# pharaofranz/frb-baseband

Hardware: AMD Instinct MI355X
Metric: Msamples/s channelised to .fil per GPU; achieved HBM GB/s vs peak (higher is better)
Workload: dtype f32

## Files before the change

### frb_baseband_amd/csrc/frbch_api.cpp

```cpp
#include "frbch_internal.h"

namespace frbchi {
int settle_user_stream(frbch_handle* h) {
  if (h->user_stream) {
    h->user_stream = 0;
    if (h->user_ev_made && dev_event_sync(h->user_ev) != 0)
      return fail(h, FRBCH_E_DEVICE, std::string("sync (caller stream): ") + dev_last_error_string());
  }
  return FRBCH_OK;
}
void mark_user_stream(frbch_handle* h, dev_stream_t s) {
  if (!h->user_ev_made) {
    if (dev_event_create_sync(&h->user_ev) != 0) return;
    h->user_ev_made = true;
  }
  dev_event_record(h->user_ev, s);
  h->user_stream = s;
}
int enter_stream(frbch_handle* h, dev_stream_t s) {
  if (h->user_stream && h->user_stream != s) { const int rc = settle_user_stream(h); if (rc) return rc; }
  join_reset(h, s);
  return FRBCH_OK;
}
void leave_stream(frbch_handle* h, dev_stream_t s) { mark_user_stream(h, s); }
// ... 18 lines not shown
  if ((cfg->flags & kFlagBuffered) && (cfg->flags & kFlagTwoPass)) return fail(h, FRBCH_E_ARG, "cfg.flags asks for the buffered AND the two-pass rescale");
  {
    const uint32_t mode = (cfg->overlap >> 24) & 0xFFu, batches = (cfg->overlap >> 16) & 0xFFu;
    if ((mode != 0 && mode != 3) || batches)
      return fail(h, FRBCH_E_ARG, "cfg.overlap: only mode 3 (or 0) and no batch count are accepted (include/frbch.h)");
  }
  h->device = cfg->device;
  DeviceGuard dg(h->device);
  char arch[128] = "";
  if (!dev_arch_ok(h->device, arch, sizeof arch, &h->lds_limit)) return fail(h, FRBCH_E_DEVICE, "cannot query device");
  h->lane_ncu = dev_cu_count(h->device);
  if (h->cfg.unpack_mode == 1) h->cfg.flags |= kFlagGenericK1;
  const std::string why = make_plan(h->cfg, &h->pl, h->lds_limit);
  if (!why.empty()) return fail(h, FRBCH_E_ARG, why);
  const Plan& pl = h->pl;
  CHECK_DEV(h, dev_stream_create(&h->stream), "hipStreamCreate");
  int rc;
  if ((rc = upload_table(h, &h->tw_r, pl.r, std::max(1, pl.r / 2), 1))) return rc;
  if ((rc = upload_table(h, &h->tw_c2, pl.c2, pl.c, 1))) return rc;
  const uint64_t nlo = 1ull << pl.log2_nlo, nhi = pl.n >> pl.log2_nlo;
  if ((rc = upload_table(h, &h->tw_nlo, pl.n, nlo, 1))) return rc;
  if ((rc = upload_table(h, &h->tw_nhi, pl.n, std::max<uint64_t>(1, nhi), nlo))) return rc;
  if ((rc = apply_plan(h))) return rc;
  CHECK_DEV(h, dev_malloc((void**)&h->s_dc, (size_t)pl.maxb * pl.c2 * sizeof(cf)), "hipMalloc(s_dc)");
  CHECK_DEV(h, dev_malloc((void**)&h->p0, (size_t)pl.maxb * pl.c2 * sizeof(cf)), "hipMalloc(p0)");
  if (pl.dls_lg_ns) {
    const std::vector<float> tab = dls_table(1u << pl.dls_lg_ns, h->cfg.dls_cutoff_sigma, h->cfg.dls_threshold);
    CHECK_DEV(h, dev_malloc((void**)&h->dls_tab, tab.size() * sizeof(float)), "hipMalloc(level table)");
    CHECK_DEV(h, dev_h2d(h->dls_tab, tab.data(), tab.size() * sizeof(float), h->stream), "upload level table");
    CHECK_DEV(h, dev_sync(h->stream), "sync");
    h->dls_cap = (((uint64_t)pl.maxb - 1) * pl.hop + pl.n) >> pl.dls_lg_ns;
    CHECK_DEV(h, dev_malloc((void**)&h->dls_nlow, h->dls_cap * sizeof(uint32_t)), "hipMalloc(window counts)");
  }
  CHECK_DEV(h, dev_malloc((void**)&h->offset, pl.ncol * sizeof(float)), "hipMalloc(offset)");
  CHECK_DEV(h, dev_malloc((void**)&h->scale, pl.ncol * sizeof(float)), "hipMalloc(scale)");
  if ((rc = set_identity_rescale(h))) return rc;
  if (pl.interval_rows == 0) {
    h->have_scale = true;
    h->scale_frozen = true;
  }
  return FRBCH_OK;
}

extern "C" void frbch_close(frbch_handle* h) {
  if (!h) return;
  DeviceGuard dg(h->device);
  (void)settle_user_stream(h);
  if (h->stream) (void)dev_sync(h->stream);
  drain_events(h);
  dev_free(h->tw_r); dev_free(h->tw_c2); dev_free(h->tw_nhi); dev_free(h->tw_nlo);
  dev_free(h->ftw1_r); dev_free(h->ftw2_r); dev_free(h->ftw1_c); dev_free(h->ftw2_c); dev_free(h->td1); dev_free(h->td2);
  dev_free(h->spill); dev_free(h->s_dc); dev_free(h->p0);
  dev_free(h->spill2); dev_free(h->chirp); dev_free(h->ptmp); dev_free(h->scr2);
  dev_free(h->offset); dev_free(h->scale); dev_free(h->powbuf); dev_free(h->partial);
  dev_free(h->d_frames); dev_free(h->d_out); dev_free(h->stg); dev_free(h->d_fbad); dev_free(h->scan_rows);
  dev_free(h->dls_tab); dev_free(h->dls_nlow);
  for (int i = 0; i < 8; ++i) { dev_host_free(h->pin_in[i]); dev_host_free(h->pin_out[i]); }
  if (h->stream) dev_stream_destroy(h->stream);
  if (h->user_ev_made) dev_event_destroy(h->user_ev);
  if (h->quant_ev_made) dev_event_destroy(h->quant_ev);
  if (h->reset_ev_made) dev_event_destroy(h->reset_ev);
  if (h->spill_ev_made) dev_event_destroy(h->spill_ev);
  for (auto& e : h->evpool) dev_event_destroy(e);
  delete h;
}

extern "C" const char* frbch_last_error(frbch_handle* h) { return h ? h->err.c_str() : "null handle"; }

extern "C" int frbch_get_info(frbch_handle* h, frbch_info* info) {
  if (!h || !info) return FRBCH_E_ARG;
  const Plan& pl = h->pl;
  memset(info, 0, sizeof *info);
  info->size = (uint32_t)sizeof *info;
  info->nchan = pl.c; info->freq_res = pl.r; info->tscrunch = pl.tscr; info->nif = pl.nif;
  info->block_samples = pl.n;
  info->block_payload_bytes = pl.block_payload_bytes;
  info->rows_per_block = pl.rows_per_block;
  info->row_bytes = pl.row_bytes;
  info->rescale_interval_rows = pl.interval_rows;
  info->rows_out = h->rows_out;
  info->blocks_done = h->blocks_done;
  info->tsamp_s = pl.tsamp_s;
  info->tstart_mjd = h->tstart_mjd;
  info->fch1_mhz = pl.fch1; info->foff_mhz = pl.foff;
  info->frame_bytes = h->have_vdif ? h->v0.frame_bytes : 0;
  info->header_bytes = h->have_vdif ? h->v0.header_bytes() : 0;
  info->have_rescale = h->have_scale ? 1 : 0;
  info->diag = h->diag;
  info->frames_seen = h->frames_seen;
  info->frames_invalid = h->frames_invalid;
  info->frame_gaps = h->frame_gaps;
  info->frames_filled = h->frames_filled;
  info->block_stride_bytes = pl.block_stride_bytes;
  info->nfilt_pos = (uint32_t)pl.nfilt_pos;
  info->nfilt_neg = (uint32_t)pl.nfilt_neg;
  return FRBCH_OK;
}

extern "C" int frbch_reset(frbch_handle* h) {
  if (!h) return FRBCH_E_ARG;
  DeviceGuard dg(h->device);
  { const int rc = settle_user_stream(h); if (rc) return rc; }
  CHECK_DEV(h, dev_sync(h->stream), "sync");
  h->pow_rows = 0;
  h->fused_rows = 0;
  h->fused_valid = false;
  h->deferred.active = false;
// ... 242 lines not shown
```

### frb_baseband_amd/csrc/frbch_internal.h

```cpp
#ifndef FRBCH_INTERNAL_H
#define FRBCH_INTERNAL_H
#include FRBCH_DEV_HEADER

#include <errno.h>
#include <fcntl.h>
#include <math.h>
#include <stdio.h>
#include <stdlib.h>
#include <string.h>
#include <sys/mman.h>
#include <sys/stat.h>
#include <sys/uio.h>
#include <time.h>
#include <unistd.h>

#include <algorithm>
#include <atomic>
#include <chrono>
#include <sstream>
#include <string>
#include <condition_variable>
#include <map>
#include <mutex>
#include <thread>
#include <vector>

#include "frbch_host.h"
#include "frbch_kparams.h"

using namespace frbch;

enum { KID_K1 = 0, KID_KC, KID_K2, KID_STATS, KID_QUANT, KID_K3, KID_K4, KID_K0, KID_K2S, KID_K2P, KID_COUNT };
const char* const kKernelNames[KID_COUNT] = {"frbch_k1_branch", "frbch_kc_dcfix", "frbch_k2_chan",
                                             "frbch_stats", "frbch_quantise", "frbch_k3_dedisp", "frbch_k4_out", "frbch_k0_stage",
                                             "frbch_k2_statpass", "frbch_k2_priv"};
static_assert(KID_COUNT <= (int)(sizeof(((frbch_timing*)nullptr)->k) / sizeof(((frbch_timing*)nullptr)->k[0])), "frbch_timing holds every slot");

struct EventPair {
  dev_event_t a, b;
  int kid;
  double bytes;
};

struct frbch_handle {
  frbch_config cfg;
  Plan pl;
  std::string err;
  int device = 0;
  dev_stream_t stream = 0;
  dev_stream_t user_stream = 0;
  dev_event_t user_ev{};
  bool user_ev_made = false;
  size_t lds_limit = 65536;

  cf *tw_r = nullptr, *tw_c2 = nullptr, *tw_nhi = nullptr, *tw_nlo = nullptr;
  cf *ftw1_r = nullptr, *ftw2_r = nullptr, *ftw1_c = nullptr, *ftw2_c = nullptr, *td1 = nullptr, *td2 = nullptr;
  cf *spill = nullptr, *s_dc = nullptr, *p0 = nullptr;
  cf *spill2 = nullptr, *chirp = nullptr;
  int coh_order_m = 0;
  float* ptmp = nullptr;
  float *offset = nullptr, *scale = nullptr;
  bool have_scale = false;
  bool scale_frozen = false;
  float* powbuf = nullptr;
  float* scr2 = nullptr;
  uint64_t pow_cap_rows = 0, pow_rows = 0;
  double* partial = nullptr;
  int partial_chunks = 0;
  uint64_t fused_rows = 0;
  bool fused_valid = false;
  int fused_chunks = 0;
  int fused_live = 0;

  uint64_t rows_out = 0, blocks_done = 0;
  struct Deferred {
    bool active = false;
    KParams p;
    uint32_t nb = 0;
    uint64_t rows = 0;
  } deferred;
  int priv_grid = 0;

  bool have_vdif = false;
  VdifInfo v0{};
  double tstart_mjd = 0.0;
  uint64_t skip_bytes = 0;
  uint64_t blocks_budget = 0;
  std::vector<uint8_t> carry;
  uint64_t frames_seen = 0, frames_invalid = 0, frame_gaps = 0, frames_filled = 0;
  std::vector<uint8_t> carry_bad;
  uint32_t* d_fbad = nullptr;
  float* dls_tab = nullptr;
  uint32_t* dls_nlow = nullptr;
  uint64_t dls_cap = 0;
  size_t d_fbad_words = 0;
  uint64_t next_frame_index = 0;
  size_t checked_bytes = 0;
  uint8_t* d_frames = nullptr;
  size_t d_frames_cap = 0;
  uint8_t* d_out = nullptr;
  size_t d_out_cap = 0;
  uint8_t* stg = nullptr;
  bool stg_ready = false;
  std::vector<uint8_t> outq;
  size_t outq_pos = 0;
  uint8_t* pin_in[8] = {nullptr, nullptr, nullptr, nullptr, nullptr, nullptr, nullptr, nullptr};
  uint8_t* pin_out[8] = {nullptr, nullptr, nullptr, nullptr, nullptr, nullptr, nullptr, nullptr};
  size_t pin_in_cap = 0, pin_out_cap = 0;
  uint8_t* sink = nullptr;
  size_t sink_line_pitch = 0;
  uint64_t sink_rows = 0, sink_rows_cap = 0;

  uint64_t out_pitch = 0;
  int lane_cus = 0;
  int lane_ncu = 0;
  bool quant_lds_allowed = false;
  dev_event_t spill_ev{};
  bool spill_ev_made = false, spill_busy = false;
  std::vector<dev_event_t> evpool;
  size_t evnext = 0;
  uint32_t diag = 0;
// ... 164 lines not shown
```

### frb_baseband_amd/csrc/frbch_kparams.h

```cpp
#ifndef FRBCH_KPARAMS_H
#define FRBCH_KPARAMS_H
#include <stdint.h>

struct __attribute__((aligned(8))) cf {
  float x, y;
};

struct __attribute__((aligned(16))) f4 {
  float v[4];
};

enum { FRBCH_OUT_FLOAT_POWER = 0, FRBCH_OUT_CODES = 1,
       FRBCH_OUT_STATS = 2 };

struct KParams {
  int log2_c2;
  int log2_r;
  int c;
  int c2;
  int r;
  int g;
  int tt;
  int tscr;
  int nif;
  int pol_mode;
  int nbit;
  int flip;
  int out_mode;
  int log2_nlo;
  int log2_g;
  int in_bits;
  uint32_t frame_bytes, header_bytes, payload_bytes;
  uint32_t rel0;
  uint64_t payload_off;
  const uint8_t* frames;
  uint64_t gs;
  cf* spill;
  cf* s_dc;
  cf* p0;
  const cf* tw_r;
  const cf* tw_c2;
  const cf* tw_nhi;
  const cf* tw_nlo;
  const cf* ftw1_r;
  const cf* ftw2_r;
  const cf* ftw1_c;
  const cf* ftw2_c;
  const cf* td1;
  const cf* td2;
  const float* offset;
  const float* scale;
  float* power_out;
  uint8_t* code_out;
  uint64_t row0;
  uint64_t out_pitch;
  uint32_t div_magic, div_shift;
  float lut[4];
  float digi_mean, digi_scale, digi_max;
  cf rot6[6];
  int coherent;
  int nfilt_pos;
  int keep;
  uint64_t hop;
  cf* spill2;
  const cf* chirp;
  float* ptmp;
  const float* scr_in;
  uint32_t scr_fact;
  uint64_t scr_rows;
  double* stat_partial;
  uint64_t stat_limit;
  uint32_t nblk;
  uint32_t stat_first;
  const uint8_t* stg;
  uint8_t* stg_out;
  int tile_major;
  const uint32_t* fbad;
  uint64_t fbad_frame0;
  uint32_t* dls_nlow;
  const float* dls_tab;
  int dls_lg_ns;
};

struct StatParams {
  const float* power;
  double* partial;
  uint64_t rows;
  uint64_t rows_per_chunk;
  int ncol, c, nif, flip, nchunk;
  int rsplit;
  int cpw;
  float* offset;
  float* scale;
};

struct QuantParams {
  const float* power;
  uint8_t* out;
  uint64_t rows;
  int ncol, c, nif, flip, nbit;
  const float* offset;
  const float* scale;
  float digi_mean, digi_scale, digi_max;
  uint32_t grid_x;
  int log2_c;
  int log2_ncol;
  uint64_t pitch;
  uint32_t rphases;
};
#define QUANT_GRID_X(p) ((p).grid_x)

struct ChirpParams {
  cf* chirp;
  int c, c2, r, log2_r;
  int usb;
  int order_m;
  double band_edge_mhz;
  double df_mhz;
  double dm_over_k;
};

#define FRBCH_CODE_INDEX(pitch, row, nif, prod, cout) ((((uint64_t)(row)) * (uint64_t)(nif) + (uint64_t)(prod)) * (uint64_t)(pitch) + (uint64_t)(cout))

#define S2_INDEX(row, pos, r) (((((uint64_t)(row) >> 2) * (uint64_t)(r) + (uint64_t)(pos)) << 2) + (uint64_t)((row) & 3))

#endif
// ... 1 lines not shown
```

### frb_baseband_amd/csrc/frbch_launch.cpp

```cpp
#include "frbch_internal.h"

#include "kernels_generic.inc"
#ifndef FRBCH_NO_FAST
#include "kernels_fast.inc"
#include "kernels_k2priv.inc"
#endif

namespace frbchi {

int upload_table(frbch_handle* h, cf** dst, uint64_t n, uint64_t count, uint64_t step) {
  std::vector<float> tmp(2 * count);
  fill_twiddles(tmp.data(), n, count, step);
  CHECK_DEV(h, dev_malloc((void**)dst, count * sizeof(cf)), "hipMalloc(twiddles)");
  CHECK_DEV(h, dev_h2d(*dst, tmp.data(), count * sizeof(cf), h->stream), "upload twiddles");
  CHECK_DEV(h, dev_sync(h->stream), "sync");
  return FRBCH_OK;
}

KParams base_params(const frbch_handle* h) {
  const Plan& pl = h->pl;
  KParams p;
  memset(&p, 0, sizeof p);
  p.log2_c2 = pl.log2_c2;
  p.log2_r = pl.log2_r;
// ... 192 lines not shown
  }
}
template <class F>
bool select_k2_fast(const Plan& pl, F&& f) {
  if (pl.fast_k2_log2m != 5) return false;
  if (pl.fast_k2_nt == 512) f(fast::frbch_k2_fast<5, 512>, ksel(512, pl.k2_fast_lds, "frbch_k2_fast", {5, 512}));
  else f(fast::frbch_k2_fast<5, 1024>, ksel(1024, pl.k2_fast_lds, "frbch_k2_fast", {5, 1024}));
  return true;
}
template <class F>
bool select_k2c_fast(const Plan& pl, F&& f) {
  return on_value<1, 2, 3, 4, 5>(pl.coh_fast_c, [&](auto L) {
    f(fast::frbch_k2c_fast<L.value, 1024>, ksel(1024, pl.k2c_fast_lds, "frbch_k2c_fast").with({L.value, 1024}));
  });
}
constexpr uint32_t kK3WaveWgs = 2048;
bool k3_wave_planned(const Plan& pl) {
  return pl.coherent && pl.coh_fast_r == 4 && pl.coh_nt == 512;
}
template <class F>
bool select_k3_fast(const Plan& pl, F&& f) {
  if (pl.coh_nt == 512) {
    if (!k3_wave_planned(pl)) return false;
    f(fast::frbch_k3_wave<4>, ksel(256, pl.k3_fast_lds, "frbch_k3_wave", {4}));
    return true;
  }
  return on_value<1, 2, 3, 5>(pl.coh_fast_r, [&](auto L) {
    f(fast::frbch_k3_fast<L.value, 1024>, ksel(1024, pl.k3_fast_lds, "frbch_k3_fast").with({L.value, 1024}));
  });
}
bool k4_fast_planned(const Plan& pl, uint32_t h_flags) {
  return pl.ncol % 64 == 0 && pl.rows_per_block % 2 == 0 && pl.c % 4 == 0 && !(h_flags & kFlagGenericK2);
}

constexpr uint32_t kFusedStatWgs = 2048;
int priv_stat_chunks(const Plan& pl, int grid) { return grid * (pl.ncol / 4 >= 256 ? 1 : (int)(256 / (pl.ncol / 4))); }
bool pol_mode_no_sums(int pol_mode) { return pol_mode == 3; }
bool priv_takes(const Plan& pl, const KParams& p, int priv_grid) {
  return pl.fast_k2_priv && p.tile_major == 2 && priv_grid > 0 &&
         !(p.out_mode == FRBCH_OUT_FLOAT_POWER && pl.fast_k2_nw == 2 && pl.fast_k2_log2m == 3);
}
struct PrivLaunch {
  unsigned grid;
  bool sums;
};
PrivLaunch priv_launch(const frbch_handle* h, const KParams& p, uint32_t nb) {
  const Plan& pl = h->pl;
  if (pl.fast_k2_lane || !priv_takes(pl, p, h->priv_grid)) return {0u, false};
  const uint64_t ntiles = (uint64_t)nb * (uint64_t)(pl.r / 4);
  const bool sums = p.stat_partial && k2_wave_planned(pl) && !pl.coherent &&
                    !pol_mode_no_sums(p.pol_mode) && !(h->cfg.flags & kFlagSeparateStats);
  return {(unsigned)std::min<uint64_t>(ntiles, (uint64_t)h->priv_grid), sums};
}
int wave_stat_chunks(const Plan& pl, uint32_t h_flags, int pol_mode) {
  if (pol_mode_no_sums(pol_mode) || pl.k2_two_stage) return 0;
  if (k3_wave_planned(pl)) return (h_flags & kFlagSeparateStats) ? 0 : (int)kK3WaveWgs;
  if (!k2_wave_planned(pl) || pl.coherent || (h_flags & kFlagSeparateStats)) return 0;
  int nt = 0;
  select_k2_wave(pl, pol_mode, false, [&](auto, const KSel& a) { nt = a.nt; });
  const int cg = (int)(pl.ncol / 4);
  if (!nt) return 0;
  if (cg > nt)
    return (cg % nt == 0 && cg / nt <= 4)
               ? (pl.fast_k2_log2m == 5 ? 256 : ((pl.fast_k2_log2m == 3 && pl.fast_k2_nw != 8) ? (int)kFusedStatWgs : 0))
               : 0;
  if (nt % cg != 0) return 0;
  return (int)kFusedStatWgs * (nt / cg);
}
int fused_stat_chunks(const Plan& pl, uint32_t h_flags, int pol_mode, int priv_grid = 0) {
  const int w = wave_stat_chunks(pl, h_flags, pol_mode);
  if (pol_mode_no_sums(pol_mode) || pl.k2_two_stage || (h_flags & kFlagSeparateStats)) return w;
  return (pl.fast_k2_priv && priv_grid > 0) ? std::max(w, priv_stat_chunks(pl, priv_grid)) : w;
}

void set_fastdiv(KParams& p) {
  const uint32_t d = p.payload_bytes;
  uint32_t l = 0;
  while ((1ull << l) < d) ++l;
  p.div_magic = (uint32_t)((((1ull << l) - d) << 32) / d + 1);
  p.div_shift = l ? l - 1 : 0;
}
bool launch_k1_wave(frbch_handle* h, KParams& p, uint32_t nb, dev_stream_t s, int ncu) {
  const Plan& pl = h->pl;
  p.nblk = nb;
  const int kg = pl.fast_k1_g;
  {
    static const int ks[6] = {1, 2, 3, 4, 8, 12};
    const int step = 64 / kg;
    for (int i = 0; i < 6; ++i) {
      const double a = -2.0 * M_PI * (double)((step * ks[i]) % pl.r) / (double)pl.r;
      p.rot6[i].x = (float)cos(a);
      p.rot6[i].y = (float)sin(a);
    }
  }
  const uint32_t ngrp = (uint32_t)(pl.c2 / kg);
  const uint32_t resident = (uint32_t)(ncu > 0 ? ncu : 256) * (uint32_t)std::max<size_t>(1, (160 * 1024) / pl.k1_fast_lds);
  uint32_t ny = std::max<uint32_t>(1, std::min<uint32_t>(nb, resident / std::max<uint32_t>(1, ngrp)));
  if (ngrp > resident && ngrp % resident != 0) {
    uint32_t g = ngrp, r = resident;
    while (r) { const uint32_t t = g % r; g = r; r = t; }
    const uint32_t want = resident / g;
    if (want <= nb) ny = want;
  }
  return select_k1_wave(pl, p.stg != nullptr, p.fbad != nullptr, [&](auto kern, const KSel& a) { launch_sel(h, kern, dim3(ngrp, ny), a, s, p); });
}
bool launch_k2_wave(frbch_handle* h, KParams& p, uint32_t nb, dev_stream_t s, uint32_t h_flags) {
// ... 47 lines not shown
  if (!pl.fast_k1_log2m) return false;
  const uint32_t rb = (uint32_t)(pl.fast_k1_wave ? pl.fast_k1_g : pl.g) / 2;
  if (p.payload_off % rb || p.payload_bytes % rb || p.header_bytes % rb || p.frame_bytes % rb ||
      ((uintptr_t)p.frames % 16))
    return false;
  if (pl.fast_k1_wave) {
    if (p.payload_bytes < 2) return false;
    const uint64_t fr0 = p.payload_off / p.payload_bytes;
    const uint64_t rel0 = p.payload_off - fr0 * p.payload_bytes;
    if (rel0 + (uint64_t)nb * pl.block_payload_bytes >= (1ull << 32)) return false;
    KParams q = p;
    q.frames = p.frames + fr0 * p.frame_bytes;
    q.rel0 = (uint32_t)rel0;
    set_fastdiv(q);
    if (h->stg_ready) q.stg = h->stg;
    h->stg_ready = false;
    if (p.fbad) {
      if (!q.stg || k1_wave_lds(pl, true) > h->lds_limit) return false;
      q.fbad_frame0 = p.fbad_frame0 + fr0;
    }
    q.tile_major = p.tile_major = pl.spill_tile_major;
    return launch_k1_wave(h, q, nb, s, h->lane_cus);
  }
  p.tile_major = pl.spill_tile_major == 8 ? 8 : 0;
  KParams q = p;
  if (h->stg_ready) q.stg = h->stg;
  h->stg_ready = false;
  {
    const uint64_t fr0 = p.payload_off / p.payload_bytes;
    const uint64_t rel0 = p.payload_off - fr0 * p.payload_bytes;
    const uint64_t span = rel0 + (uint64_t)(nb - 1) * pl.block_stride_bytes + pl.block_payload_bytes;
    if (p.payload_bytes >= 2 && span < (1ull << 32)) {
      q.frames = p.frames + fr0 * p.frame_bytes;
      q.rel0 = (uint32_t)rel0;
      q.payload_off = rel0;
      set_fastdiv(q);
    } else {
      q.div_magic = 0;
    }
  }
  return select_k1_fast(pl, [&](auto kern, const KSel& a) { launch_sel(h, kern, dim3(pl.c2 / pl.g, nb), a, s, q); });
}
bool launch_k2_fast(frbch_handle* h, KParams& p, uint32_t nb, dev_stream_t s) {
  const Plan& pl = h->pl;
  if (pl.fast_k2_lane) {
    if (p.tile_major) return false;
    const dim3 grid((unsigned)((uint64_t)pl.r * nb * pl.fast_k2_lane / 256));
    return select_k2_lane(pl, p.pol_mode, [&](auto kern, const KSel& a) { launch_sel(h, kern, grid, a, s, p); });
  }
  if (const PrivLaunch pv = priv_launch(h, p, nb); pv.grid) {
    p.nblk = nb;
    if (!pv.sums) p.stat_partial = nullptr;
    if (!p.stat_partial) p.stat_first = 0;
    const dim3 grid(pv.grid);
    return select_k2_priv(pl, p.pol_mode, p.out_mode, [&](auto kern, const KSel& a) { launch_sel(h, kern, grid, a, s, p); });
  }
  if (p.out_mode == FRBCH_OUT_STATS) return false;
  if (!pl.fast_k2_wave && pl.fast_k2_log2m != 5) return false;
  KParams q = p;
  if (pl.k2_two_stage) {
    q.tscr = pl.k2_stage1_tscr;
    q.out_mode = FRBCH_OUT_FLOAT_POWER;
    q.power_out = h->scr2;
    q.row0 = 0;
    q.stat_partial = nullptr;
  }
  KParams& k = pl.k2_two_stage ? q : p;
  if (pl.fast_k2_wave) {
    if (!launch_k2_wave(h, k, nb, s, h->cfg.flags)) return false;
  } else {
    select_k2_fast(pl, [&](auto kern, const KSel& a) {
      launch_sel(h, kern, dim3(pl.r / (a.nt == 512 ? 1 : std::max(2, k.tscr)), nb), a, s, k);
    });
  }
  if (pl.k2_two_stage) {
    p.scr_in = h->scr2;
    p.scr_fact = (uint32_t)pl.k2_two_stage;
    p.scr_rows = (uint64_t)nb * pl.rows_per_block;
    p.stat_partial = nullptr;
    const uint64_t groups = p.scr_rows * (uint64_t)(pl.ncol / 4);
    const unsigned gx = (unsigned)std::min<uint64_t>((groups + 255) / 256, 8192);
    if (h->profiling) note_launch(h, "frbch_k2_scrunch", gx, 1);
    hipLaunchKernelGGL(fast::frbch_k2_scrunch, dim3(gx), dim3(256), 0, s, p);
  }
  return true;
}
bool launch_k2c_fast(frbch_handle* h, KParams& p, uint32_t nb, dev_stream_t s) {
  const Plan& pl = h->pl;
  if (!pl.coh_fast_c) return false;
  const int tt = 1024 / (16 << pl.coh_fast_c);
  p.nblk = nb;
  const uint32_t ntile = (uint32_t)(pl.r / tt);
  const uint32_t want = 4u * (uint32_t)std::max(1, h->lane_ncu);
  const uint32_t gy = std::max<uint32_t>(1, std::min<uint32_t>(nb, (want + ntile - 1) / ntile));
  return select_k2c_fast(pl, [&](auto kern, const KSel& a) { launch_sel(h, kern, dim3(ntile, gy), a, s, p); });
}
bool launch_k3_fast(frbch_handle* h, KParams& p, uint32_t nb, dev_stream_t s) {
  const Plan& pl = h->pl;
  if (!pl.coh_fast_r || !h->coh_order_m) return false;
  if (k3_wave_planned(pl)) {
    const uint64_t ntiles = (uint64_t)nb * pl.c;
    return select_k3_fast(pl, [&](auto kern, const KSel& a) {
      p.nblk = nb;
      launch_sel(h, kern, dim3((unsigned)std::min<uint64_t>(ntiles, kK3WaveWgs)), a, s, p);
    });
  }
// ... 141 lines not shown
  const Plan& pl = h->pl;
  p.tile_major = 0;
  if (pl.dls_lg_ns) {
    const int rc = launch_dls_count(h, p, ((uint64_t)nb - 1) * pl.hop + pl.n, s);
    if (rc) return rc;
  }
  {
    const bool masked = p.fbad != nullptr;
    if (!masked || pl.fast_k1_wave) launch_k0_stage(h, p, nb, s);
    const double bytes = (double)nb * ((double)pl.block_payload_bytes * p.frame_bytes / p.payload_bytes +
                                       (double)pl.n * 8.0 + (double)pl.c2 * 8.0);
    ProfScope ps(h, s, KID_K1, bytes);
    bool done = false;
    if (masked && !(pl.fast_k1_wave && (!pl.coherent || h->coh_order_m) && (done = launch_k1_fast(h, p, nb, s)))) {
      h->stg_ready = false;
      if (pl.coherent && h->coh_order_m) {
        const int rc = build_chirp(h, 0);
        if (rc) return rc;
      }
    } else if (masked) {
    } else if (!pl.coherent) done = launch_k1_fast(h, p, nb, s);
    else if (h->coh_order_m) {
      done = launch_k1_fast(h, p, nb, s);
      if (!done) {
        const int rc = build_chirp(h, 0);
        if (rc) return rc;
      }
    }
    if (!done) {
      REC_LAUNCH(h, frbch_k1_branch, pl.c2 / pl.g, nb, pl.nthreads, pl.k1_lds, s, p);
      if (!h->kname[KID_K1].empty() && h->kname[KID_K1].find(kKernelNames[KID_K1]) == std::string::npos)
        h->kname[KID_K1] += std::string("+") + kKernelNames[KID_K1];
    }
  }
  if (!pl.coherent) {
    ProfScope ps(h, s, KID_KC, (double)nb * pl.c2 * 16.0);
    if (!launch_kc_fast(h, p, nb, s)) REC_LAUNCH(h, frbch_kc_dcfix, 1, nb, pl.nthreads, pl.kc_lds, s, p);
  }
  CHECK_DEV(h, dev_check_launch(), "launch K1/Kc");
  return FRBCH_OK;
}

int launch_back(frbch_handle* h, KParams& p, uint32_t nb, dev_stream_t s) {
  const Plan& pl = h->pl;
  const int tile_t = std::max(pl.tt, pl.tscr);
  const double out_b = p.out_mode == FRBCH_OUT_FLOAT_POWER ? (double)pl.ncol * 4.0 : (double)pl.row_bytes;
  const double bytes = (double)nb * ((double)pl.n * 8.0 + (double)pl.rows_per_block * out_b);
#ifndef FRBCH_NO_FAST
  const bool k3_sums = k3_wave_planned(pl) && h->coh_order_m != 0;
#else
  const bool k3_sums = false;
#endif
  if ((!k2_wave_planned(pl) || pl.coherent) && !k3_sums) p.stat_partial = nullptr;
  if (p.out_mode == FRBCH_OUT_STATS) {
    ProfScope ps(h, s, KID_K2S, (double)nb * (double)pl.n * 8.0);
    if (!launch_k2_fast(h, p, nb, s)) return fail(h, FRBCH_E_STATE, "statistics-only K2 pass without frbch_k2_priv");
    CHECK_DEV(h, dev_check_launch(), "launch K2 (statistics pass)");
    return FRBCH_OK;
  }
  if (pl.coherent) {
    {
      ProfScope ps(h, s, KID_K2, ((double)nb * 16.0 + (pl.coh_fast_c ? 1.0 : (double)nb) * 8.0) * (double)pl.n);
      if (!launch_k2c_fast(h, p, nb, s)) REC_LAUNCH(h, frbch_k2c_chirp, pl.r / pl.tt, nb, pl.nthreads, pl.k2_lds, s, p);
    }
    {
      ProfScope ps(h, s, KID_K3, (double)nb * ((double)pl.n * 8.0 + (double)pl.rows_per_block * pl.ncol * 4.0));
      if (!launch_k3_fast(h, p, nb, s)) REC_LAUNCH(h, frbch_k3_dedisp, pl.c, nb, pl.nthreads, pl.k3_lds, s, p);
    }
    {
      ProfScope ps(h, s, KID_K4, (double)nb * (double)pl.rows_per_block * (pl.ncol * 4.0 + out_b));
      const int tc = pl.ncol < 64 ? (int)pl.ncol : 64;
      const int gx = (int)((pl.rows_per_block + 63) / 64) * (int)(pl.ncol / tc);
#ifndef FRBCH_NO_FAST
      if (k4_fast_planned(pl, h->cfg.flags)) {
        if (h->profiling) note_launch(h, "frbch_k4_fast", gx, nb);
        hipLaunchKernelGGL(fast::frbch_k4_fast, dim3(gx, nb), dim3(256), 0, s, p);
      } else
#endif
      REC_LAUNCH(h, frbch_k4_out, gx, nb, pl.nthreads, pl.k4_lds, s, p);
    }
    CHECK_DEV(h, dev_check_launch(), "launch K2c/K3/K4");
    return FRBCH_OK;
  }
#ifndef FRBCH_NO_FAST
  const int kid = priv_takes(pl, p, h->priv_grid) ? KID_K2P : KID_K2;
#else
  const int kid = KID_K2;
#endif
  ProfScope ps(h, s, kid, bytes);
  if (!launch_k2_fast(h, p, nb, s)) REC_LAUNCH(h, frbch_k2_chan, pl.r / tile_t, nb, pl.nthreads, pl.k2_lds, s, p);
  CHECK_DEV(h, dev_check_launch(), "launch K2");
  return FRBCH_OK;
}

int ensure_partial(frbch_handle* h) {
  if (h->partial) return FRBCH_OK;
  const Plan& pl = h->pl;
  h->partial_chunks = (int)std::min<uint64_t>(32768, std::max<uint64_t>(2048, (8ull << 20) / (pl.ncol * 16)));
  h->fused_chunks = 0;
#ifndef FRBCH_NO_FAST
  h->fused_chunks = fused_stat_chunks(pl, h->cfg.flags, h->cfg.pol_mode, h->priv_grid);
#endif
  const size_t chunks = (size_t)std::max(h->partial_chunks, h->fused_chunks);
  CHECK_DEV(h, dev_malloc((void**)&h->partial, chunks * pl.ncol * 2 * sizeof(double)), "hipMalloc(partials)");
  return FRBCH_OK;
}
int clear_partial(frbch_handle* h, KParams& p, uint32_t nb, dev_stream_t s) {
  const Plan& pl = h->pl;
  int own = 0;
#ifndef FRBCH_NO_FAST
  if (const PrivLaunch pv = priv_launch(h, p, nb); pv.sums) own = priv_stat_chunks(pl, (int)pv.grid);
#endif
  p.stat_first = own ? 1u : 0u;
  h->fused_live = own;
  return own ? FRBCH_OK : extend_partial(h, s);
}
int extend_partial(frbch_handle* h, dev_stream_t s) {
  if (h->fused_live >= h->fused_chunks) return FRBCH_OK;
  const size_t row_bytes = (size_t)h->pl.ncol * 2 * sizeof(double);
  if (dev_memset((char*)h->partial + (size_t)h->fused_live * row_bytes, 0, (size_t)(h->fused_chunks - h->fused_live) * row_bytes, s) != 0)
    return fail(h, FRBCH_E_DEVICE, "clear partial sums");
  h->fused_live = h->fused_chunks;
  return FRBCH_OK;
}
int ensure_powbuf(frbch_handle* h) {
  const int rc = ensure_partial(h);
  if (rc || h->powbuf) return rc;
  const Plan& pl = h->pl;
  h->pow_cap_rows = pl.interval_rows + (uint64_t)pl.maxb * pl.rows_per_block;
  CHECK_DEV(h, dev_malloc((void**)&h->powbuf, h->pow_cap_rows * pl.ncol * sizeof(float)), "hipMalloc(power buffer)");
  return FRBCH_OK;
}

static int stat_final_cpw(const Plan& pl) { return pl.ncol < 1024 ? 2 : 8; }

int run_stats(frbch_handle* h, uint64_t rows, dev_stream_t s) {
  const Plan& pl = h->pl;
  StatParams sp;
  memset(&sp, 0, sizeof sp);
  if (h->fused_valid && h->fused_chunks && h->fused_rows == rows) {
    sp.partial = h->partial;
    sp.rows = rows;
    sp.ncol = (int)pl.ncol;
    sp.c = pl.c;
    sp.nif = pl.nif;
    sp.flip = pl.flip;
    sp.nchunk = h->fused_live;
    sp.cpw = stat_final_cpw(pl);
    sp.offset = h->offset;
    sp.scale = h->scale;
    ProfScope ps(h, s, KID_STATS, (double)h->fused_live * pl.ncol * 16.0);
    REC_LAUNCH(h, frbch_stats_final, (int)((pl.ncol + sp.cpw - 1) / sp.cpw), 1, 256, 256 * 2 * sizeof(double), s, sp);
    CHECK_DEV(h, dev_check_launch(), "launch stats (final)");
    return FRBCH_OK;
  }
  if (!h->powbuf) return fail(h, FRBCH_E_STATE, "rescale statistics: neither fused sums nor buffered rows");
  sp.power = h->powbuf;
// ... 81 lines not shown
        }
        if (h->profiling) note_launch(h, "frbch_quantise_fast<8, 512>", qp.grid_x, 1);
        hipLaunchKernelGGL((fast::frbch_quantise_fast<8, 512>), dim3(qp.grid_x), dim3(512), kHold, s, qp);
      } else {
        if (h->profiling) note_launch(h, "frbch_quantise_fast<8, 256>", qp.grid_x, 1);
        hipLaunchKernelGGL((fast::frbch_quantise_fast<8, 256>), dim3(qp.grid_x), dim3(256), 0, s, qp);
      }
      CHECK_DEV(h, dev_check_launch(), "launch quantise");
      return FRBCH_OK;
    }
  }
#endif
  REC_LAUNCH(h, frbch_quantise, qp.grid_x, 1, 256, 0, s, qp);
  CHECK_DEV(h, dev_check_launch(), "launch quantise");
  return FRBCH_OK;
}

uint64_t out_row_span(const frbch_handle* h) {
  const Plan& pl = h->pl;
  if (!h->out_pitch) return pl.row_bytes;
  const uint64_t bits = pl.row_bytes * 8 / pl.ncol;
  return h->out_pitch * (uint64_t)pl.nif * bits / 8;
}
uint64_t out_extent(const frbch_handle* h, uint64_t rows) {
  const Plan& pl = h->pl;
  if (!rows) return 0;
  if (!h->out_pitch) return rows * pl.row_bytes;
  const uint64_t bits = pl.row_bytes * 8 / pl.ncol;
  const uint64_t line = h->out_pitch * bits / 8, seg = (uint64_t)pl.c * bits / 8;
  return (rows * pl.nif - 1) * line + seg;
}


int allow_generic_lds(frbch_handle* h) {
  const Plan& pl = h->pl;
  CHECK_DEV(h, dev_allow_lds(frbch_k1_branch, pl.k1_lds), "LDS size K1");
  CHECK_DEV(h, dev_allow_lds(frbch_k2_chan, pl.k2_lds), "LDS size K2");
  CHECK_DEV(h, dev_allow_lds(frbch_kc_dcfix, pl.kc_lds), "LDS size Kc");
  if (pl.coherent) {
    CHECK_DEV(h, dev_allow_lds(frbch_k2c_chirp, pl.k2_lds), "LDS size K2c");
    CHECK_DEV(h, dev_allow_lds(frbch_k3_dedisp, pl.k3_lds), "LDS size K3");
  }
  return FRBCH_OK;
}

int apply_plan(frbch_handle* h) {
  const Plan& pl = h->pl;
  cf** const tables[] = {&h->ftw1_r, &h->ftw2_r, &h->ftw1_c, &h->ftw2_c, &h->td1, &h->td2, &h->spill, &h->spill2, &h->chirp};
  for (cf** t : tables) { dev_free(*t); *t = nullptr; }
  dev_free(h->stg); h->stg = nullptr; h->stg_ready = false;
  dev_free(h->scr2); h->scr2 = nullptr;
  dev_free(h->ptmp); h->ptmp = nullptr;
  dev_free(h->partial); h->partial = nullptr;
  h->partial_chunks = h->fused_chunks = 0;
  h->fused_rows = 0;
  h->fused_valid = false;
  for (std::string& n : h->kname) n.clear();
  h->launch_rec.clear();
  int rc;
  if ((rc = allow_generic_lds(h))) return rc;
  h->priv_grid = pl.fast_k2_priv ? 2 * std::max(1, h->lane_ncu) : 0;
  if ((rc = setup_fast(h))) return rc;
  CHECK_DEV(h, dev_malloc((void**)&h->spill, (size_t)pl.maxb * (pl.c2 / pl.g) * pl.gs * sizeof(cf)), "hipMalloc(spill)");
#ifndef FRBCH_NO_FAST
  if (pl.k2_two_stage)
    CHECK_DEV(h, dev_malloc((void**)&h->scr2, (size_t)pl.maxb * (pl.r / pl.k2_stage1_tscr) * pl.ncol * sizeof(float)), "hipMalloc(tscrunch scratch)");
#endif
  if (pl.coherent) {
    CHECK_DEV(h, dev_malloc((void**)&h->spill2, (size_t)pl.maxb * pl.n * sizeof(cf)), "hipMalloc(spill2)");
    CHECK_DEV(h, dev_malloc((void**)&h->chirp, (size_t)pl.n * sizeof(cf)), "hipMalloc(chirp)");
    CHECK_DEV(h, dev_malloc((void**)&h->ptmp, (size_t)pl.maxb * pl.rows_per_block * pl.ncol * sizeof(float)), "hipMalloc(ptmp)");
    if ((rc = build_chirp(h, pl.coh_fast_r ? (1 << pl.coh_fast_r) : 0))) return rc;
    if (h->kname[KID_K2].empty()) h->kname[KID_K2] = "frbch_k2c_chirp";
  }
  return FRBCH_OK;
}

int fused_chunks_of(const frbch_handle* h) {
#ifndef FRBCH_NO_FAST
  return fused_stat_chunks(h->pl, h->cfg.flags, h->cfg.pol_mode, h->priv_grid);
#else
  (void)h;
  return 0;
#endif
}

int launch_unpack_tap(frbch_handle* h, KParams& p, uint64_t nsamples, int decoder, dev_stream_t s) {
  if (h->pl.dls_lg_ns) {
    if (decoder != 0) return fail(h, FRBCH_E_ARG, "dynamic level setting is decoded by the generic unpack only");
    const int rc = launch_dls_count(h, p, nsamples, s);
    if (rc) return rc;
  }
  if (decoder == 0) {
    REC_LAUNCH(h, frbch_unpack_tap, (nsamples + 255) / 256, 1, 256, 0, s, p);
  } else {
#ifndef FRBCH_NO_FAST
    if (h->profiling) note_launch(h, "frbch_unpack_tap_fast", (nsamples / 2 + 255) / 256, 1);
    hipLaunchKernelGGL(fast::frbch_unpack_tap_fast, dim3((unsigned)((nsamples / 2 + 255) / 256)), dim3(256), 0, s, p);
#else
    return fail(h, FRBCH_E_ARG, "the register kernels are not part of this build");
#endif
  }
  CHECK_DEV(h, dev_check_launch(), "launch unpack tap");
  return FRBCH_OK;
}

// ... 2 lines not shown
```

### frb_baseband_amd/csrc/kernels_k2priv.inc

```

namespace fast {

enum { K2P_CODES = 0, K2P_POWER = 1, K2P_STATS = 2 };
constexpr uint32_t kK2PFlushMask = 7u;
constexpr int kK2PQReads = 8;
#ifndef FI
#define FI __device__ __forceinline__
#endif

constexpr int kK2PrivSeq = 2048 + 2048 / 8;
constexpr size_t k2_priv_lds_bytes() { return (size_t)4 * kK2PrivSeq * sizeof(cf) + (size_t)1024 * sizeof(cf); }

template <int PM, int MODE>
__global__ void __launch_bounds__(256, 2) frbch_k2_priv(KParams p) {
  constexpr int LOG2M = 3;
  using GE = GeoW<LOG2M, 1>;
  constexpr int M = GE::M, C2 = GE::L, C = C2 / 2, TPS = GE::TPS, SEQ = kK2PrivSeq, LPS = GE::LPS, VT = GE::VT;
  static_assert(M == 8 && C2 == 2048 && TPS == 128 && LPS == 64 && VT == 2, "written for 2C = 2048");
  constexpr int NW = 4, NT = 64 * NW, TT = NW, ROT = 32 / M;
  constexpr int LG_TT = 2;
  constexpr int NIF = PM >= 4 ? 4 : 1, NCOL = NIF * C, NG = NCOL / 4;
  constexpr int CGT = NG >= NT ? NG / NT : 1;
  constexpr int RS = NG >= NT ? 1 : NT / NG;
  constexpr int GL = 8;
// ... 5 lines not shown
  const int ql = lane;
  cf* const s = lds + wave * SEQ;

  const int lg_tpb = p.log2_r - LG_TT;
  const uint32_t ntiles = p.nblk << lg_tpb;
  const uint32_t nwg = gridDim.x, wg = blockIdx.x;
  const uint32_t per = ntiles / nwg, extra = ntiles % nwg;
  const uint32_t first = wg * per + (wg < extra ? wg : extra);
  const uint32_t count = per + (wg < extra ? 1u : 0u);
  if (!count) return;

  if (gridDim.x > 1 && blockIdx.x >= (gridDim.x + 1) / 2) __builtin_amdgcn_s_sleep(127);

  RegTw<LOG2M, VT> rtw;
  rtw.load(p.ftw1_c, p.ftw2_c, ql, LPS, TPS);

  const uint32_t ng = (uint32_t)(C2 / GL);
  const uint32_t loff = (uint32_t)((lane >> 3) * (2 * GL) + (lane & 7));
  cf v[VT][16];
  auto tile_base = [&](uint32_t tile) {
    const uint32_t b_ = tile >> lg_tpb, t_ = ((tile & ((1u << lg_tpb) - 1u)) << LG_TT) + (uint32_t)wave;
    return p.spill + (uint64_t)b_ * (uint64_t)ng * p.gs + (uint64_t)(t_ >> 1) * (uint64_t)(2 * C2) + (uint64_t)((t_ & 1u) * GL);
  };
  auto load_reg = [&](const cf* base, const int vt, const int a) {
    const nf2 t2 = *reinterpret_cast<const nf2*>(base + (size_t)(a * 16 * 2 * GL + vt * 8 * 2 * GL) + loff);
    v[vt][a] = cf{t2.x, t2.y};
  };
  auto load_tile = [&](uint32_t tile) {
    const cf* base = tile_base(tile);
#pragma unroll
    for (int vt = 0; vt < VT; ++vt)
#pragma unroll
      for (int a = 0; a < 16; ++a) load_reg(base, vt, a);
  };
  load_tile(first);

  const int rph = RS > 1 ? tid / NG : 0;
  float4 of4[CGT], sc4[CGT];
#pragma unroll
  for (int g = 0; g < CGT; ++g) of4[g] = sc4[g] = make_float4(0.f, 0.f, 0.f, 0.f);
  const int flip = p.flip;
  if constexpr (MODE == K2P_CODES) {
#pragma unroll
    for (int g = 0; g < CGT; ++g) {
      const int col0 = ((RS > 1 ? tid % NG : tid) + NT * g) * 4, prod = col0 / C, cout0 = col0 - prod * C;
      const int kbase = flip ? (C - 4 - cout0) : cout0;
      of4[g] = *reinterpret_cast<const float4*>(p.offset + prod * C + kbase);
      sc4[g] = *reinterpret_cast<const float4*>(p.scale + prod * C + kbase);
    }
  }
  const bool stat_on = MODE != K2P_CODES && p.stat_partial != nullptr;
  const int lg_t = 31 - __builtin_clz(p.tscr);
  const int R = p.r;
  auto flush_sums = [&](const bool fresh) {
    int tl = tid;
    asm volatile("" : "+v"(tl));
    typedef double nd2 __attribute__((ext_vector_type(2)));
    constexpr int GB = CGT >= 2 ? 2 : 1;
    const bool fl = MODE == K2P_STATS && flip;
#pragma unroll
    for (int g0 = 0; g0 < CGT; g0 += GB) {
      nd2 cur[GB][4];
#pragma unroll
      for (int gg = 0; gg < GB; ++gg) {
        const int g = g0 + gg;
        const nd2* src = reinterpret_cast<const nd2*>(p.stat_partial + (((size_t)blockIdx.x * RS + (RS > 1 ? tl / NG : 0)) * NCOL + (size_t)((RS > 1 ? tl % NG : tl) + NT * g) * 4) * 2);
#pragma unroll
        for (int e = 0; e < 4; ++e) cur[gg][e] = nd2{0.0, 0.0};
        if (MODE != K2P_STATS || !fresh)
#pragma unroll
          for (int e = 0; e < 4; ++e) cur[gg][e] = src[e];
      }
#pragma unroll
      for (int gg = 0; gg < GB; ++gg) {
        const int g = g0 + gg;
        nd2* dst = reinterpret_cast<nd2*>(p.stat_partial + (((size_t)blockIdx.x * RS + (RS > 1 ? tl / NG : 0)) * NCOL + (size_t)((RS > 1 ? tl % NG : tl) + NT * g) * 4) * 2);
        const float a1[4] = {fl ? of4[g].w : of4[g].x, fl ? of4[g].z : of4[g].y, fl ? of4[g].y : of4[g].z, fl ? of4[g].x : of4[g].w};
        const float a2[4] = {fl ? sc4[g].w : sc4[g].x, fl ? sc4[g].z : sc4[g].y, fl ? sc4[g].y : sc4[g].z, fl ? sc4[g].x : sc4[g].w};
#pragma unroll
        for (int e = 0; e < 4; ++e) {
          nd2 t = cur[gg][e];
          t.x = (fresh ? 0.0 : t.x) + (double)a1[e];
          t.y = (fresh ? 0.0 : t.y) + (double)a2[e];
          dst[e] = t;
        }
        of4[g] = sc4[g] = make_float4(0.f, 0.f, 0.f, 0.f);
      }
      __builtin_amdgcn_sched_barrier(0);
    }
  };
  int cur_blk = -1;
  __builtin_amdgcn_s_waitcnt(0x0F70);

  for (uint32_t it = 0; it < count; ++it) {
    const uint32_t tile = first + it;
    const int blk = (int)(tile >> lg_tpb);
    const int t0 = (int)(tile & ((1u << lg_tpb) - 1u)) << LG_TT;
    if (blk != cur_blk) {
      cur_blk = blk;
      const cf* dP = p.p0 + (size_t)blk * C2 + C;
      int tl = tid;
      asm volatile("" : "+v"(tl));
#pragma unroll
      for (int i = 0; i < C / NT; ++i) dpl[pw_swz(tl + NT * i, ROT)] = dP[tl + NT * i];
      __syncthreads();
    }

    __builtin_amdgcn_s_setprio(1);
    fwd_passes_w<LOG2M, 1, VT, true>(v, s, ql, p.ftw1_c, p.ftw2_c, &rtw);

    const cf* const nbase = tile_base(it + 1 < count ? tile + 1 : tile);
#pragma unroll
    for (int vt = 0; vt < VT; ++vt) {
      const int q = ql + LPS * vt;
      const int k0 = (q / M) + 16 * (q % M);
      static_assert((2 * ROT * (TPS / 32)) % 32 == 0 && TPS % 32 == 0, "pw_swz(k + 2 TPS) == pw_swz(k) + 2 TPS");
      const int ks0 = pw_swz(k0, ROT), ks1 = pw_swz(k0 + TPS, ROT);
      cf2* dst = reinterpret_cast<cf2*>(s + q * 18 + 8);
#pragma unroll
      for (int i = 0; i < 4; ++i) {
        const cf a = add(v[vt][8 + 2 * i], dpl[ks0 + 2 * TPS * i]);
        const cf b = add(v[vt][9 + 2 * i], dpl[ks1 + 2 * TPS * i]);
        dst[i] = cf2{a, b};
        __builtin_amdgcn_sched_barrier(0);
        load_reg(nbase, vt, 8 + 2 * i);
        load_reg(nbase, vt, 9 + 2 * i);
        __builtin_amdgcn_sched_barrier(0);
      }
    }
    cf wm[VT][8];
#pragma unroll
    for (int vt = 0; vt < VT; ++vt) {
      const int q = ql + LPS * vt;
      const cf2* src = reinterpret_cast<const cf2*>(s + (TPS - 1 - q) * 18 + 8);
#pragma unroll
      for (int i = 0; i < 4; ++i) {
        const cf2 t = src[i];
        wm[vt][7 - 2 * i] = t.a;
        wm[vt][6 - 2 * i] = t.b;
      }
    }
// ... 77 lines not shown
            const nf4 o4 = {t.x, t.y, t.z, t.w};
            __builtin_nontemporal_store(o4, reinterpret_cast<nf4*>(p.power_out + orow * (uint64_t)NCOL + col0));
          }
          if (!decltype(chk)::value || (stat_on && orow < p.stat_limit)) {
            of4[g].x += t.x; of4[g].y += t.y; of4[g].z += t.z; of4[g].w += t.w;
            sc4[g].x = fmaf(t.x, t.x, sc4[g].x); sc4[g].y = fmaf(t.y, t.y, sc4[g].y);
            sc4[g].z = fmaf(t.z, t.z, sc4[g].z); sc4[g].w = fmaf(t.w, t.w, sc4[g].w);
          }
        }
      };
      auto row_ptr = [&](const int t, const int g) {
        const int col0 = (cg0 + NT * g) * 4, prod = col0 / C, cout0 = col0 - prod * C;
        const int kb = flip ? (C - 4 - cout0) : cout0;
        return reinterpret_cast<const float4*>(reinterpret_cast<const float*>(lds + (size_t)t * SEQ) + prod * C + pw_swz(kb, ROT));
      };
      bool all_in = true, none_in = false;
      if constexpr (MODE == K2P_STATS) {
        const uint64_t lim = stat_on ? p.stat_limit : 0;
        all_in = row_base + (uint64_t)rows_out <= lim;
        none_in = row_base >= lim;
      }
      using Chk = std::integral_constant<bool, MODE != K2P_STATS>;
      if (lg_t == 0 && (MODE != K2P_CODES || nbit == 8) && all_in) {
        constexpr int NR = TT / RS;
        constexpr int QR = (NR * CGT > kK2PQReads) ? (kK2PQReads / CGT > 0 ? kK2PQReads / CGT : 1) : NR;
#pragma unroll
        for (int j0 = 0; j0 < NR; j0 += QR) {
          float4 acc[QR][CGT];
#pragma unroll
          for (int jj = 0; jj < QR; ++jj)
#pragma unroll
            for (int g = 0; g < CGT; ++g) acc[jj][g] = *row_ptr(rph + RS * (j0 + jj), g);
#pragma unroll
          for (int jj = 0; jj < QR; ++jj)
#pragma unroll
            for (int g = 0; g < CGT; ++g) emit_group(acc[jj][g], g, row_base + (uint64_t)(rph + RS * (j0 + jj)), Chk());
        }
      } else if (!none_in) {
        for (int j = rph; j < rows_out; j += RS) {
#pragma unroll
          for (int g = 0; g < CGT; ++g) {
            float4 acc = *row_ptr(j << lg_t, g);
            for (int tt = 1; tt < T; ++tt) {
              const float4 x = *row_ptr((j << lg_t) + tt, g);
              acc.x += x.x; acc.y += x.y; acc.z += x.z; acc.w += x.w;
            }
            emit_group(acc, g, row_base + (uint64_t)j, std::true_type());
          }
        }
      }
    }
    __syncthreads();
    if constexpr (MODE != K2P_CODES) {
      if (stat_on && ((it & kK2PFlushMask) == kK2PFlushMask || it + 1 == count)) flush_sums(p.stat_first && it <= kK2PFlushMask);
    }
  }

}

}
```

Before: 150,300.

## Stage periodic rescale-sum flushes in float slices and fold once at kernel end

Each periodic flush of per-workgroup offset/scale sums used to read, add and rewrite a row of double-precision partials in global memory. Now every flush writes only float4 slices to its own slot in a new per-workgroup buffer, and a single fold at the end of the kernel adds all slots into the double partial row. This removes the read-modify-write traffic and its dependency from the main tile loop. In exchange it needs an extra allocation sized by the worst-case flush count, adds a capacity check that can fail a launch, and gives up double accumulation between flushes.

Result: faster. 152,400, median of 6 (+1.4%).

```diff
diff --git a/frb_baseband_amd/csrc/frbch_api.cpp b/frb_baseband_amd/csrc/frbch_api.cpp
--- a/frb_baseband_amd/csrc/frbch_api.cpp
+++ b/frb_baseband_amd/csrc/frbch_api.cpp
@@ -94,7 +94,7 @@
   dev_free(h->ftw1_r); dev_free(h->ftw2_r); dev_free(h->ftw1_c); dev_free(h->ftw2_c); dev_free(h->td1); dev_free(h->td2);
   dev_free(h->spill); dev_free(h->s_dc); dev_free(h->p0);
   dev_free(h->spill2); dev_free(h->chirp); dev_free(h->ptmp); dev_free(h->scr2);
-  dev_free(h->offset); dev_free(h->scale); dev_free(h->powbuf); dev_free(h->partial);
+  dev_free(h->offset); dev_free(h->scale); dev_free(h->powbuf); dev_free(h->partial); dev_free(h->stat_slices);
   dev_free(h->d_frames); dev_free(h->d_out); dev_free(h->stg); dev_free(h->d_fbad); dev_free(h->scan_rows);
   dev_free(h->dls_tab); dev_free(h->dls_nlow);
   for (int i = 0; i < 8; ++i) { dev_host_free(h->pin_in[i]); dev_host_free(h->pin_out[i]); }
diff --git a/frb_baseband_amd/csrc/frbch_internal.h b/frb_baseband_amd/csrc/frbch_internal.h
--- a/frb_baseband_amd/csrc/frbch_internal.h
+++ b/frb_baseband_amd/csrc/frbch_internal.h
@@ -67,6 +67,8 @@
   uint64_t pow_cap_rows = 0, pow_rows = 0;
   double* partial = nullptr;
   int partial_chunks = 0;
+  float* stat_slices = nullptr;
+  uint32_t stat_slots = 0;
   uint64_t fused_rows = 0;
   bool fused_valid = false;
   int fused_chunks = 0;
diff --git a/frb_baseband_amd/csrc/frbch_kparams.h b/frb_baseband_amd/csrc/frbch_kparams.h
--- a/frb_baseband_amd/csrc/frbch_kparams.h
+++ b/frb_baseband_amd/csrc/frbch_kparams.h
@@ -72,6 +72,8 @@
   uint64_t stat_limit;
   uint32_t nblk;
   uint32_t stat_first;
+  float* stat_slices;
+  uint32_t stat_slots;
   const uint8_t* stg;
   uint8_t* stg_out;
   int tile_major;
diff --git a/frb_baseband_amd/csrc/frbch_launch.cpp b/frb_baseband_amd/csrc/frbch_launch.cpp
--- a/frb_baseband_amd/csrc/frbch_launch.cpp
+++ b/frb_baseband_amd/csrc/frbch_launch.cpp
@@ -268,6 +268,12 @@
                     !pol_mode_no_sums(p.pol_mode) && !(h->cfg.flags & kFlagSeparateStats);
   return {(unsigned)std::min<uint64_t>(ntiles, (uint64_t)h->priv_grid), sums};
 }
+uint32_t priv_stat_slots(const Plan& pl, uint32_t nb, unsigned grid) {
+  if (!grid) return 0;
+  const uint64_t ntiles = (uint64_t)nb * (uint64_t)(pl.r / 4);
+  const uint64_t trips = (ntiles + grid - 1) / grid;
+  return (uint32_t)((trips + fast::kK2PFlushMask) / (fast::kK2PFlushMask + 1u));
+}
 int wave_stat_chunks(const Plan& pl, uint32_t h_flags, int pol_mode) {
   if (pol_mode_no_sums(pol_mode) || pl.k2_two_stage) return 0;
   if (k3_wave_planned(pl)) return (h_flags & kFlagSeparateStats) ? 0 : (int)kK3WaveWgs;
@@ -421,6 +427,8 @@
     p.nblk = nb;
     if (!pv.sums) p.stat_partial = nullptr;
     if (!p.stat_partial) p.stat_first = 0;
+    p.stat_slices = p.stat_partial ? h->stat_slices : nullptr;
+    p.stat_slots = p.stat_partial ? h->stat_slots : 0u;
     const dim3 grid(pv.grid);
     return select_k2_priv(pl, p.pol_mode, p.out_mode, [&](auto kern, const KSel& a) { launch_sel(h, kern, grid, a, s, p); });
   }
@@ -668,6 +676,11 @@
   const bool k3_sums = false;
 #endif
   if ((!k2_wave_planned(pl) || pl.coherent) && !k3_sums) p.stat_partial = nullptr;
+#ifndef FRBCH_NO_FAST
+  if (const PrivLaunch pv = priv_launch(h, p, nb); pv.sums && (!h->stat_slices || priv_stat_slots(pl, nb, pv.grid) > h->stat_slots))
+    return fail(h, FRBCH_E_CAPACITY, "frbch_k2_priv: " + std::to_string(priv_stat_slots(pl, nb, pv.grid)) + " flushes per workgroup, " +
+                                         std::to_string(h->stat_slots) + " slots of rescale sums allocated");
+#endif
   if (p.out_mode == FRBCH_OUT_STATS) {
     ProfScope ps(h, s, KID_K2S, (double)nb * (double)pl.n * 8.0);
     if (!launch_k2_fast(h, p, nb, s)) return fail(h, FRBCH_E_STATE, "statistics-only K2 pass without frbch_k2_priv");
@@ -719,6 +732,13 @@
 #endif
   const size_t chunks = (size_t)std::max(h->partial_chunks, h->fused_chunks);
   CHECK_DEV(h, dev_malloc((void**)&h->partial, chunks * pl.ncol * 2 * sizeof(double)), "hipMalloc(partials)");
+#ifndef FRBCH_NO_FAST
+  h->stat_slots = 0;
+  if (pl.fast_k2_priv && h->priv_grid > 0 && !pol_mode_no_sums(h->cfg.pol_mode) && !(h->cfg.flags & kFlagSeparateStats)) {
+    h->stat_slots = priv_stat_slots(pl, (uint32_t)pl.maxb, (unsigned)h->priv_grid);
+    CHECK_DEV(h, dev_malloc((void**)&h->stat_slices, (size_t)h->priv_grid * h->stat_slots * pl.ncol * 2 * sizeof(float)), "hipMalloc(slices of partials)");
+  }
+#endif
   return FRBCH_OK;
 }
 int clear_partial(frbch_handle* h, KParams& p, uint32_t nb, dev_stream_t s) {
@@ -906,6 +926,8 @@
   dev_free(h->scr2); h->scr2 = nullptr;
   dev_free(h->ptmp); h->ptmp = nullptr;
   dev_free(h->partial); h->partial = nullptr;
+  dev_free(h->stat_slices); h->stat_slices = nullptr;
+  h->stat_slots = 0;
   h->partial_chunks = h->fused_chunks = 0;
   h->fused_rows = 0;
   h->fused_valid = false;
diff --git a/frb_baseband_amd/csrc/kernels_k2priv.inc b/frb_baseband_amd/csrc/kernels_k2priv.inc
--- a/frb_baseband_amd/csrc/kernels_k2priv.inc
+++ b/frb_baseband_amd/csrc/kernels_k2priv.inc
@@ -81,41 +81,54 @@
   const bool stat_on = MODE != K2P_CODES && p.stat_partial != nullptr;
   const int lg_t = 31 - __builtin_clz(p.tscr);
   const int R = p.r;
-  auto flush_sums = [&](const bool fresh) {
+  static_assert(MODE == K2P_CODES || RS == 1, "the slices hold one row of sums per workgroup");
+  auto flush_sums = [&](const uint32_t k) {
     int tl = tid;
     asm volatile("" : "+v"(tl));
+    const bool fl = MODE == K2P_STATS && flip;
+    float* const sl = p.stat_slices + ((uint64_t)blockIdx.x * (uint64_t)p.stat_slots + (uint64_t)k) * (uint64_t)(2 * NCOL);
+#pragma unroll
+    for (int g = 0; g < CGT; ++g) {
+      const uint64_t col = (uint64_t)(tl + NT * g) * 4u;
+      const nf4 a1 = {fl ? of4[g].w : of4[g].x, fl ? of4[g].z : of4[g].y, fl ? of4[g].y : of4[g].z, fl ? of4[g].x : of4[g].w};
+      const nf4 a2 = {fl ? sc4[g].w : sc4[g].x, fl ? sc4[g].z : sc4[g].y, fl ? sc4[g].y : sc4[g].z, fl ? sc4[g].x : sc4[g].w};
+      *reinterpret_cast<nf4*>(sl + col) = a1;
+      *reinterpret_cast<nf4*>(sl + (uint64_t)NCOL + col) = a2;
+      of4[g] = sc4[g] = make_float4(0.f, 0.f, 0.f, 0.f);
+    }
+  };
+  auto fold_sums = [&](const uint32_t nflush) {
     typedef double nd2 __attribute__((ext_vector_type(2)));
-    constexpr int GB = CGT >= 2 ? 2 : 1;
-    const bool fl = MODE == K2P_STATS && flip;
-#pragma unroll
-    for (int g0 = 0; g0 < CGT; g0 += GB) {
-      nd2 cur[GB][4];
-#pragma unroll
-      for (int gg = 0; gg < GB; ++gg) {
-        const int g = g0 + gg;
-        const nd2* src = reinterpret_cast<const nd2*>(p.stat_partial + (((size_t)blockIdx.x * RS + (RS > 1 ? tl / NG : 0)) * NCOL + (size_t)((RS > 1 ? tl % NG : tl) + NT * g) * 4) * 2);
-#pragma unroll
-        for (int e = 0; e < 4; ++e) cur[gg][e] = nd2{0.0, 0.0};
-        if (MODE != K2P_STATS || !fresh)
-#pragma unroll
-          for (int e = 0; e < 4; ++e) cur[gg][e] = src[e];
-      }
-#pragma unroll
-      for (int gg = 0; gg < GB; ++gg) {
-        const int g = g0 + gg;
-        nd2* dst = reinterpret_cast<nd2*>(p.stat_partial + (((size_t)blockIdx.x * RS + (RS > 1 ? tl / NG : 0)) * NCOL + (size_t)((RS > 1 ? tl % NG : tl) + NT * g) * 4) * 2);
-        const float a1[4] = {fl ? of4[g].w : of4[g].x, fl ? of4[g].z : of4[g].y, fl ? of4[g].y : of4[g].z, fl ? of4[g].x : of4[g].w};
-        const float a2[4] = {fl ? sc4[g].w : sc4[g].x, fl ? sc4[g].z : sc4[g].y, fl ? sc4[g].y : sc4[g].z, fl ? sc4[g].x : sc4[g].w};
-#pragma unroll
-        for (int e = 0; e < 4; ++e) {
-          nd2 t = cur[gg][e];
-          t.x = (fresh ? 0.0 : t.x) + (double)a1[e];
-          t.y = (fresh ? 0.0 : t.y) + (double)a2[e];
-          dst[e] = t;
-        }
-        of4[g] = sc4[g] = make_float4(0.f, 0.f, 0.f, 0.f);
-      }
-      __builtin_amdgcn_sched_barrier(0);
+    constexpr uint32_t kFoldSlots = 4;
+    const float* const sl0 = p.stat_slices + (uint64_t)blockIdx.x * (uint64_t)p.stat_slots * (uint64_t)(2 * NCOL);
+    const bool fresh = p.stat_first != 0;
+    for (int g = 0; g < CGT; ++g) {
+      const uint64_t col = (uint64_t)(tid + NT * g) * 4u;
+      nd2* const row = reinterpret_cast<nd2*>(p.stat_partial + ((uint64_t)blockIdx.x * (uint64_t)NCOL + col) * 2u);
+      nd2 acc[4];
+#pragma unroll
+      for (int e = 0; e < 4; ++e) acc[e] = fresh ? nd2{0.0, 0.0} : row[e];
+      for (uint32_t k0 = 0; k0 < nflush; k0 += kFoldSlots) {
+        nf4 a1[kFoldSlots], a2[kFoldSlots];
+#pragma unroll
+        for (uint32_t j = 0; j < kFoldSlots; ++j) {
+          const uint32_t k = k0 + j < nflush ? k0 + j : nflush - 1u;
+          const float* const sl = sl0 + (uint64_t)k * (uint64_t)(2 * NCOL) + col;
+          a1[j] = *reinterpret_cast<const nf4*>(sl);
+          a2[j] = *reinterpret_cast<const nf4*>(sl + NCOL);
+        }
+#pragma unroll
+        for (uint32_t j = 0; j < kFoldSlots; ++j) {
+          if (k0 + j < nflush) {
+            acc[0].x += (double)a1[j].x; acc[0].y += (double)a2[j].x;
+            acc[1].x += (double)a1[j].y; acc[1].y += (double)a2[j].y;
+            acc[2].x += (double)a1[j].z; acc[2].y += (double)a2[j].z;
+            acc[3].x += (double)a1[j].w; acc[3].y += (double)a2[j].w;
+          }
+        }
+      }
+#pragma unroll
+      for (int e = 0; e < 4; ++e) row[e] = acc[e];
     }
   };
   int cur_blk = -1;
@@ -299,10 +312,13 @@
     }
     __syncthreads();
     if constexpr (MODE != K2P_CODES) {
-      if (stat_on && ((it & kK2PFlushMask) == kK2PFlushMask || it + 1 == count)) flush_sums(p.stat_first && it <= kK2PFlushMask);
+      if (stat_on && ((it & kK2PFlushMask) == kK2PFlushMask || it + 1 == count)) flush_sums(it >> 3);
     }
   }
-
+  if constexpr (MODE != K2P_CODES) {
+    static_assert(kK2PFlushMask == 7u, "slot = trip / 8");
+    if (stat_on) fold_sums((count + kK2PFlushMask) >> 3);
+  }
 }
 
 }
```
